# sair-lab/AirSLAM

Hardware: AMD Instinct MI355X
Metric: stereo detect+match pairs/sec (2x PLNet @512x512 internal: points + lines, junctions on the left + LightGlue match) (higher is better)
Workload: dtype fp16

## Files before the change

### airslam_amd/_lib.py

```python
from __future__ import annotations

import ctypes as C
import os

_HERE = os.path.dirname(os.path.abspath(__file__))
LIB_PATH = os.path.join(_HERE, "libairfe.so")


class Tuning(C.Structure):
    _fields_ = [(n, C.c_int) for n in (
        "fuse_lg_block", "gemm_small_max_m", "gemm8_min_m", "gemmr_min_m", "gemmr_wgs", "qkv_pair", "block_min_m", "lgb_tokens", "sg_kenc_gemm",
        "fold_qkv", "overlap_lines", "kf_graph", "kf_spec_rows", "fuse_dec", "assign_fused", "fold_out_proj", "desc_gather_stream", "copy_wgs")] + [("reserved", C.c_int * 5)]


class Cfg(C.Structure):
    _fields_ = [
        ("device", C.c_int), ("precision", C.c_int), ("max_batch", C.c_int), ("enc_chunk", C.c_int),
        ("max_keypoints", C.c_int), ("keypoint_threshold", C.c_float), ("remove_borders", C.c_int),
        ("nms_radius", C.c_int), ("line_threshold", C.c_float), ("line_length_threshold", C.c_float),
        ("matcher", C.c_int), ("image_width", C.c_int), ("image_height", C.c_int), ("sinkhorn_iters", C.c_int),
        ("superpoint_pack", C.c_char_p), ("plnet_s1_pack", C.c_char_p), ("lightglue_pack", C.c_char_p),
        ("superglue_pack", C.c_char_p), ("matcher_precision", C.c_int), ("line_precision", C.c_int), ("check_launches", C.c_int),
        ("tuning", C.POINTER(Tuning)),
    ]
# ... 262 lines not shown
    "airfe_debug_line_mid": (C.c_int, [C.c_void_p, C.POINTER(DebugLineMidArgs)]),
    "airfe_debug_s0_decode": (C.c_int, [C.c_void_p, C.POINTER(DebugS0DecodeArgs)]),
    "airfe_debug_lg_prepare": (C.c_int, [C.c_void_p, C.POINTER(DebugLgPrepareArgs)]),
    "airfe_debug_lg_assign": (C.c_int, [C.c_void_p, C.POINTER(DebugLgAssignArgs)]),
    "airfe_debug_plnet_stage0": (C.c_int, [C.c_void_p] + [C.c_void_p] * 10),
    "airfe_debug_plnet_s1": (C.c_int, [C.c_void_p, C.POINTER(Stage0), C.c_void_p, C.c_void_p, C.c_int, C.POINTER(C.c_int)]),
    "airfe_debug_plnet_s1_last": (C.c_int, [C.c_void_p, C.c_void_p, C.c_void_p, C.c_int, C.POINTER(C.c_int)]),
    "airfe_debug_preprocess": (C.c_int, [C.c_void_p, C.c_void_p, C.c_int, C.c_int, C.c_int, C.c_void_p]),
    "airfe_debug_conv3x3": (C.c_int, [C.c_void_p, C.c_void_p, C.c_int, C.c_int, C.c_int, C.c_int, C.c_void_p, C.c_void_p,
                                      C.c_int, C.c_int, C.c_void_p]),
    "airfe_debug_conv": (C.c_int, [C.c_void_p, C.POINTER(DebugConvArgs)]),
    "airfe_debug_trace": (C.c_int, [C.c_void_p, C.c_int]),
    "airfe_debug_trace_stop": (C.c_int, [C.c_void_p, C.c_int]),
    "airfe_debug_trace_buffer": (C.c_int, [C.c_void_p, C.c_int, C.c_void_p, C.c_size_t]),
    "airfe_debug_trace_slots": (C.c_int, [C.c_void_p]),
    "airfe_debug_trace_slot": (C.c_int, [C.c_void_p, C.c_int, C.c_char_p, C.c_int, C.POINTER(C.c_uint), C.POINTER(C.c_uint), C.POINTER(C.c_uint)]),
    "airfe_debug_trace_read": (C.c_int, [C.c_void_p, C.c_void_p, C.c_void_p, C.c_void_p]),
    "airfe_debug_gemm": (C.c_int, [C.c_void_p, C.c_void_p, C.c_int, C.c_int, C.c_void_p, C.c_void_p, C.c_int, C.c_int,
                                   C.c_void_p]),
    "airfe_debug_linear": (C.c_int, [C.c_void_p, C.POINTER(DebugLinearArgs)]),
    "airfe_debug_qkv": (C.c_int, [C.c_void_p] + [C.c_int] * 3 + [C.c_void_p] * 3 + [C.c_int] + [C.c_void_p] * 4 + [C.c_int] * 2 + [C.c_void_p] * 3),
    "airfe_debug_lg_block": (C.c_int, [C.c_void_p, C.POINTER(DebugLgBlockArgs)]),
    "airfe_debug_ln_gelu": (C.c_int, [C.c_void_p, C.c_int, C.c_void_p, C.c_void_p, C.c_void_p, C.c_int]),
    "airfe_debug_attention_args": (C.c_int, [C.c_void_p, C.POINTER(DebugAttentionArgs)]),
    "airfe_debug_attention": (C.c_int, [C.c_void_p, C.c_void_p, C.c_void_p, C.c_void_p, C.c_void_p, C.c_int, C.c_int, C.c_int, C.c_int, C.c_void_p]),
}

_lib = None


# ... 19 lines not shown
```

### airslam_amd/api.py

```python
from __future__ import annotations

import ctypes as C
import os
import tempfile
from typing import Dict, Optional

import numpy as np

from . import _lib, weights as W

FEAT = 259


def _pack_arg(x, tmpfiles) -> Optional[bytes]:
    if x is None:
        return None
    if isinstance(x, (str, bytes, os.PathLike)):
        return os.fsencode(x)
    f = tempfile.NamedTemporaryFile(suffix=".airfe", delete=False)
    f.close()
    W.save_pack(f.name, x)
    tmpfiles.append(f.name)
    return f.name.encode()


class AirfeError(RuntimeError):
    pass


class Context:

    def __init__(self, superpoint=None, lightglue=None, superglue=None, plnet_s1=None, tuning=None, **cfg):
        self._l = _lib.lib()
        c = _lib.Cfg()
        self._l.airfe_default_cfg(C.byref(c))
        t = None
        if tuning:
            t = _lib.Tuning()
            self._l.airfe_default_tuning(C.byref(t))
            for k, v in tuning.items():
                if k == "reserved" or not hasattr(t, k):
                    raise TypeError(f"unknown airfe_tuning field {k!r}")
                setattr(t, k, int(v))
            c.tuning = C.pointer(t)
        for k, v in cfg.items():
            if not hasattr(c, k):
                raise TypeError(f"unknown airfe_cfg field {k!r}")
            setattr(c, k, v)
        tmp = []
        try:
            c.superpoint_pack = _pack_arg(superpoint, tmp)
# ... 1296 lines not shown
```

### airslam_amd/csrc/airfe_debug.hip

```cpp
#include "airfe_host.h"

#include <memory>

struct HookStage {
  enum { OWN_TEXT = 1, SATURATION = 2, DEVICE_WIDE = 4 };
  HookStage(airfe_ctx* c_, const std::string& who_, int pack_prec = 0) : c(c_), who(who_), st(c_->stream) { mem.pack_prec = pack_prec; }
  HookStage(const HookStage&) = delete;
  ~HookStage() {
    if (queued) (void)hipStreamSynchronize(st);
    for (void* p : mem.allocs) (void)hipFree(p);
  }
  int status() const { return rc; }
  hipStream_t stream() { queued = true; return st; }
  int refuse(const std::string& m) { return rc ? rc : rc = fail(c, who + ": " + m); }
  void step(int r) { queued = true; if (r) rc = 1; }
  template <class T> T* fresh(size_t n, int byte) {
    T* p = raw<T>(n);
    fill(p, byte, std::max<size_t>(n, 1) * sizeof(T));
    return p;
  }
  template <class T> T* up(std::vector<T> v) { T* p = raw<T>(v.size()); put(p, std::move(v)); return p; }
  template <class T> T* up(const T* src, size_t n) { return up(std::vector<T>(src, src + n)); }
  bool linear(const float* W, const float* b, int K, int N, LinW& out) { if (!rc && !make_linear(&mem, W, b, K, N, out)) refuse("allocation failed"); return !rc; }
  void fill(void* p, int byte, size_t bytes) { if (!rc && bytes) hip(hipMemsetAsync(p, byte, bytes, stream()), "hipMemsetAsync"); }
// ... 174 lines not shown
  } else {
    g.X = s.up(dbg_conv_x(a->x, B, cin, H, W, prec));
  }
  g.Wp = s.up(dbg_conv_slabs(a->w, cin, cout, prec));
  g.bias = s.up(a->b, (size_t)cout);
  uint16_t* dy = s.fresh<uint16_t>(total, 0xFF);
  if (s.status()) return 1;
  g.Y = dy + guard;
  g.B = B; g.H = H; g.W = W; g.CIN = cin; g.COUT = cout; g.pool = pool; g.out_pad = opad; g.relu = a->relu; g.wgs = a->wgs;
  if (fused) launch_conv64r(prec, g, s.stream());
  else launch_conv3x3(prec, g, s.stream());
  s.wait(HookStage::OWN_TEXT);
  s.get(a->y_raw, dy, total * 2);
  return s.status();
} AIRFE_CATCH(c)

int airfe_debug_linear(airfe_ctx* c, const airfe_debug_linear_args* a) try {
  AIRFE_ENTER(c);
  if (!a || !a->x1 || !a->w || !a->b || !a->out) return fail(c, "debug_linear: null argument");
  const int prec = a->prec, M = a->M, K = a->K, N = a->N, epi = a->epi, kern = a->kernel, K1 = a->x2 ? a->K1 : K;
  if ((prec != 0 && prec != 1) || M < 1 || N < 1 || (K != 128 && K != 256 && K != 512) || K1 < 32 || K1 % 32 || K1 > K || (a->x2 && K1 == K) ||
      epi < EPI_STORE || epi > EPI_SOFTMAX_D2S || kern < AIRFE_DEBUG_KERNEL_DISPATCH || kern > AIRFE_DEBUG_KERNEL_GEMMR_GATHER128 || (a->act != ACT_NONE && a->act != ACT_RELU))
    return fail(c, "debug_linear: bad argument");
  const bool trans = epi == EPI_HEADS_T, heads = epi == EPI_HEADS || trans, d2s = epi == EPI_SOFTMAX_D2S;
  if (heads && ((a->H != 4 && a->H != 0) || a->Np < 16 || a->Np % 16 || M % a->Np || (epi == EPI_HEADS ? (N != 256 && N != 512) || (N == 512 && !a->out2) : N != 256)))
    return fail(c, "debug_linear: head layouts need H = 4, M = S * Np with Np a multiple of 16, N = 256 (or 512 with out2 for EPI_HEADS)");
  if ((a->rot_cos || a->rot_sin) && (epi != EPI_HEADS || !a->rot_cos || !a->rot_sin)) return fail(c, "debug_linear: rotary is an EPI_HEADS form");
  if (epi == EPI_RESID && (!a->x32 || N % 64)) return fail(c, "debug_linear: EPI_RESID needs x32 and N a multiple of 64");
  if (d2s && (K != 256 || N != 65 || a->x2 || a->rowidx || a->act || a->d2s_hc < 1 || a->d2s_wc < 1 || M % (a->d2s_hc * a->d2s_wc) || M % 16 ||
              (kern != AIRFE_DEBUG_KERNEL_DISPATCH && kern != AIRFE_DEBUG_KERNEL_GEMM8)))
// ... 890 lines not shown
```

### airslam_amd/csrc/common.h

```cpp
#pragma once
#include <hip/hip_runtime.h>
#include <stdint.h>
#include <atomic>
#include <mutex>

namespace airfe {

struct PerDeviceOnce {
  std::atomic<bool> done[64] = {};
  std::mutex mu;
  struct Token {
    PerDeviceOnce* owner = nullptr;
    int dev = 0;
    bool yes = false;
    std::unique_lock<std::mutex> lock;
    Token() = default;
    Token(Token&& o) noexcept : owner(o.owner), dev(o.dev), yes(o.yes), lock(std::move(o.lock)) { o.owner = nullptr; }
    Token(const Token&) = delete;
    Token& operator=(const Token&) = delete;
    explicit operator bool() const { return yes; }
    ~Token() { if (owner) owner->done[dev].store(true, std::memory_order_release); }
  };
  Token first() {
    Token t;
// ... 162 lines not shown
}

__device__ __forceinline__ void rotate_pairs(float* v, const f32x4& c, const f32x4& s) {
#pragma unroll
  for (int i = 0; i < 4; ++i) {
    float t0, t1, r0, r1;
    asm("v_mul_f32 %0, %1, %2" : "=v"(t0) : "v"(v[2 * i + 1]), "v"(s[i]));
    asm("v_fma_f32 %0, %1, %2, -%3" : "=v"(r0) : "v"(v[2 * i]), "v"(c[i]), "v"(t0));
    asm("v_mul_f32 %0, %1, %2" : "=v"(t1) : "v"(v[2 * i]), "v"(s[i]));
    asm("v_fma_f32 %0, %1, %2, %3" : "=v"(r1) : "v"(v[2 * i + 1]), "v"(c[i]), "v"(t1));
    v[2 * i] = r0;
    v[2 * i + 1] = r1;
  }
}

__device__ __forceinline__ void tile_decode(int tile, int per_img, int tiles_x, int sh_img, int sh_x, int& b, int& ty, int& tx) {
  if (sh_img >= 0) {
    b = tile >> sh_img;
    const int rem = tile & (per_img - 1);
    ty = rem >> sh_x;
    tx = rem & (tiles_x - 1);
  } else {
    b = tile / per_img;
    const int rem = tile - b * per_img;
    ty = rem / tiles_x;
    tx = rem - ty * tiles_x;
  }
}

__device__ __forceinline__ float wave_sum(float v) {
#pragma unroll
  for (int o = 32; o > 0; o >>= 1) v += __shfl_xor(v, o);
  return v;
}
__device__ __forceinline__ float wave_max(float v) {
#pragma unroll
  for (int o = 32; o > 0; o >>= 1) v = fmaxf(v, __shfl_xor(v, o));
  return v;
}

}
```

### airslam_amd/csrc/kernels.h

```cpp
#pragma once
#include <hip/hip_runtime.h>
#include <stdint.h>

namespace airfe {

enum Epi {
  EPI_STORE = 0,
  EPI_STORE_F32 = 1,
  EPI_RESID = 2,
  EPI_HEADS = 3,
  EPI_HEADS_T = 4,
  EPI_SOFTMAX_D2S = 5
};
enum Act { ACT_NONE = 0, ACT_RELU = 1 };

struct GemmArgs {
  const uint16_t* X1 = nullptr;
  const uint16_t* X2 = nullptr;
  int ld1 = 0, ld2 = 0, K1 = 0;
  const uint16_t* Wp = nullptr;
  const float* bias = nullptr;
  int M = 0;
  int N = 0;
  int cb_total = 0;
// ... 48 lines not shown
  const uint16_t* Wp = nullptr;
  const float* bias = nullptr;
  uint16_t* Y = nullptr;
  int B = 0, H = 0, W = 0, CIN = 0, COUT = 0;
  int pool = 0;
  int out_pad = 1;
  int relu = 1;
  int wgs = 256;
  const float* img = nullptr;
  const float* w1a = nullptr;
  const float* b1a = nullptr;
};
void launch_conv3x3(int prec, const ConvArgs& a, hipStream_t st);
void launch_conv64r(int prec, const ConvArgs& a, hipStream_t st);
void launch_conv128r(int prec, const ConvArgs& a, hipStream_t st);

void launch_preprocess(const uint8_t* src, int B, int h, int w, int stride, size_t img_stride,
                       const int* xtab , const int* ytab , const float* lut ,
                       float* out, int RH, int RW, hipStream_t st, const uint8_t* src1 = nullptr, int n0 = 0);

void launch_remap_linear(const uint8_t* src, int B, int h, int w, int stride, size_t img_stride, const float* mapx, const float* mapy,
                         uint8_t* dst, int dstride, size_t dimg_stride, hipStream_t st);

void launch_softmax_d2s(const float* logits, int ldl, float* heat, int B, int HC, int WC, hipStream_t st);
void launch_l2norm256(float* d, int rows, hipStream_t st);
void launch_simple_nms(const float* heat, float* out, float* tmp, int B, int H, int W, int radius, hipStream_t st);
void launch_nms512_candidates(const float* heat, float* out, void* planes, int B, float thr, int border, unsigned long long* cand,
                              int* cand_cnt, int cand_cap, hipStream_t st);
void launch_candidates(const float* heat, int B, int H, int W, float thr, int border, unsigned long long* cand,
                       int* cand_cnt, int cand_cap, hipStream_t st);
// ... 418 lines not shown
```

### airslam_amd/csrc/kernels_conv128r.hip

```cpp
#include "common.h"
#include "kernels.h"

namespace airfe {

typedef __attribute__((address_space(3))) void* las_ptr128r;

__device__ __forceinline__ void c128r_glds16(const void* gsrc, unsigned lds_off) {
  unsigned keep;
  asm volatile("s_mov_b32 %0, m0\n\ts_mov_b32 m0, %2\n\ts_nop 0\n\tglobal_load_lds_dwordx4 %1, off\n\ts_mov_b32 m0, %0"
               : "=&s"(keep)
               : "v"(gsrc), "s"(lds_off)
               : "memory");
}

constexpr int C128R_TILE_BYTES = 10 * 18 * 256;
constexpr int C128R_PIECES = 10 * 18 * 16;
constexpr int C128R_OUT_OFF = 2 * C128R_TILE_BYTES;
constexpr int C128R_LDS = C128R_OUT_OFF + 128 * 256;

template <class P, bool POOL>
__global__ __launch_bounds__(512, 1) void conv128r_kernel(ConvArgs a, int tiles_x, int tiles_y, int ntiles, int cb0) {
  extern __shared__ __attribute__((aligned(16))) char smem[];
  const int tid = threadIdx.x, lane = tid & 63, l15 = lane & 15, g = lane >> 4;
  const int wave = __builtin_amdgcn_readfirstlane(tid >> 6);
  const int cb = cb0 + (wave >> 2), t = wave & 3;
  const int H = a.H, W = a.W, COUT = a.COUT;
  const size_t in_row = (size_t)(W + 2) * 256;
  const size_t in_img = (size_t)(H + 2) * in_row;
  const int per_img = tiles_x * tiles_y;
  const unsigned lds_base = __builtin_amdgcn_readfirstlane((unsigned)(size_t)(las_ptr128r)smem);

  typename P::vec8 wreg[9][2][2];
  {
    const char* wp = reinterpret_cast<const char*>(a.Wp) + (size_t)cb * 18 * SLAB_BYTES;
    const int rr = t * 16 + l15;
#pragma unroll
    for (int tap = 0; tap < 9; ++tap)
#pragma unroll
      for (int cc = 0; cc < 2; ++cc)
#pragma unroll
        for (int ks = 0; ks < 2; ++ks) {
          const uint4 u = *reinterpret_cast<const uint4*>(wp + (tap * 2 + cc) * SLAB_BYTES + rr * 128 + (((ks * 4 + g) ^ swz128(rr)) << 4));
          wreg[tap][cc][ks] = __builtin_bit_cast(typename P::vec8, u);
        }
  }
  const int f0 = (t >> 1) * 32 + g * 8 + (t & 1) * 4;
  const f32x4 bias = *reinterpret_cast<const f32x4*>(a.bias + cb * 64 + f0);

  int goff[6];
#pragma unroll
  for (int j = 0; j < 6; ++j) {
    const int q = min(j * 512 + tid, C128R_PIECES - 1);
    const int p = q >> 4;
    const int pr = p / 18, pc = p - pr * 18;
    const int c = (q & 15) ^ (pc & 15);
    goff[j] = pr * (int)in_row + pc * 256 + c * 16;
  }
  const bool last_piece = 5 * 512 + tid < C128R_PIECES;
  auto stage_tile = [&](int tile, int buf) {
    const int b = tile / per_img, rem = tile - b * per_img;
    const int ty = rem / tiles_x, tx = rem - ty * tiles_x;
    const char* xin = reinterpret_cast<const char*>(a.X) + (size_t)b * in_img + (size_t)ty * 8 * in_row + (size_t)tx * 16 * 256;
    const unsigned dst = lds_base + buf * C128R_TILE_BYTES + wave * 1024;
#pragma unroll
    for (int j = 0; j < 5; ++j) c128r_glds16(xin + goff[j], dst + j * 8192);
    if (last_piece) c128r_glds16(xin + goff[5], dst + 5 * 8192);
  };
  int cbase[3];
#pragma unroll
  for (int dx = 0; dx < 3; ++dx) cbase[dx] = (l15 + dx) * 256 + ((g ^ ((l15 + dx) & 15)) << 4);

  const int Ho = POOL ? H / 2 : H, Wo = POOL ? W / 2 : W;
  const int opad = a.out_pad;
  const size_t orow = (size_t)(Wo + 2 * opad) * COUT;
  char* ost = smem + C128R_OUT_OFF;

  int tile = blockIdx.x;
  if (tile < ntiles) stage_tile(tile, 0);
  asm volatile("s_waitcnt vmcnt(0)" ::: "memory");
  __syncthreads();

  for (int i = 0; tile < ntiles; ++i, tile += gridDim.x) {
    const int next = tile + gridDim.x;
    if (next < ntiles) stage_tile(next, (i + 1) & 1);
    const int xoff = (i & 1) * C128R_TILE_BYTES;
    f32x4 acc[8];
#pragma unroll
    for (int m = 0; m < 8; ++m) acc[m] = bias;
#pragma unroll
    for (int c = 0; c < 12; ++c) {
      const int dx = c >> 2, cc = (c >> 1) & 1, ks = c & 1;
      typename P::vec8 bf[10];
      const char* fb = smem + ((cbase[dx] ^ (ks << 6) ^ (cc << 7)) + xoff);
#pragma unroll
      for (int r = 0; r < 10; ++r) bf[r] = lds_frag<P>(fb, r * (18 * 256));
#pragma unroll
      for (int dy = 0; dy < 3; ++dy)
#pragma unroll
        for (int m = 0; m < 8; ++m) acc[m] = P::mfma(wreg[dy * 3 + dx][cc][ks], bf[m + dy], acc[m]);
    }
    asm volatile("s_waitcnt vmcnt(0)" ::: "memory");
    __syncthreads();

    const int b = tile / per_img, rem = tile - b * per_img;
    const int ty = rem / tiles_x, tx = rem - ty * tiles_x;
    uint16_t* ybase = a.Y + (size_t)b * (Ho + 2 * opad) * orow + cb0 * 64;
    const int fch = (wave >> 2) * 8 + (f0 >> 3);
    uint2 pk[8];
#pragma unroll
    for (int m = 0; m < 8; ++m) pk[m] = uint2{P::pack2(acc[m][0], acc[m][1]), P::pack2(acc[m][2], acc[m][3])};
    if constexpr (!POOL) {
#pragma unroll
      for (int m = 0; m < 8; ++m) {
        const int px = m * 16 + l15;
        uint2 v = pk[m];
        if (a.relu) { v.x = relu_packed(v.x); v.y = relu_packed(v.y); }
        *reinterpret_cast<uint2*>(ost + px * 256 + ((fch ^ (px & 15)) << 4) + (t & 1) * 8) = v;
      }
      __syncthreads();
#pragma unroll
// ... 14 lines not shown
        if (a.relu) { v.x = relu_packed(v.x); v.y = relu_packed(v.y); }
        const int px = mp * 8 + (l15 >> 1);
        if (!(l15 & 1)) *reinterpret_cast<uint2*>(ost + px * 256 + ((fch ^ (px & 15)) << 4) + (t & 1) * 8) = v;
      }
      __syncthreads();
      {
        const int q = tid, px = q >> 4, c = q & 15;
        const uint4 v = *reinterpret_cast<const uint4*>(ost + px * 256 + ((c ^ (px & 15)) << 4));
        const int y = ty * 4 + (px >> 3), x = tx * 8 + (px & 7);
        *reinterpret_cast<uint4*>(ybase + (size_t)(y + opad) * orow + (size_t)(x + opad) * COUT + c * 8) = v;
      }
    }
  }
}

template <class P, bool POOL>
static void conv128r_launch_t(const ConvArgs& a, hipStream_t st) {
  static PerDeviceOnce attr_once;
  auto kfn = conv128r_kernel<P, POOL>;
  if (auto once_token = attr_once.first()) {
    (void)hipFuncSetAttribute(reinterpret_cast<const void*>(kfn), hipFuncAttributeMaxDynamicSharedMemorySize, C128R_LDS);
  }
  const int tiles_x = a.W / 16, tiles_y = a.H / 8;
  const int ntiles = tiles_x * tiles_y * a.B;
  const int grid = ntiles < a.wgs ? ntiles : a.wgs;
  for (int cb0 = 0; cb0 < a.COUT / 64; cb0 += 2)
    hipLaunchKernelGGL(kfn, dim3(grid), dim3(512), C128R_LDS, st, a, tiles_x, tiles_y, ntiles, cb0);
}

void launch_conv128r(int prec, const ConvArgs& a, hipStream_t st) {
  if (prec == 1) {
    if (a.pool) conv128r_launch_t<PF16, true>(a, st); else conv128r_launch_t<PF16, false>(a, st);
  } else {
    if (a.pool) conv128r_launch_t<PBF16, true>(a, st); else conv128r_launch_t<PBF16, false>(a, st);
  }
}

}
```

### airslam_amd/csrc/kernels_conv64r.hip

```cpp
#include "common.h"
#ifdef C64R_TIMING
__device__ long long c64_dbg[256 * 8 * 6];
#define C64R_T(x) { const long long now_ = wall_clock64(); x += now_ - tp_; tp_ = now_; }
#else
#define C64R_T(x)
#endif
#include "kernels.h"

namespace airfe {

typedef __attribute__((address_space(3))) void* las_ptr64r;

__device__ __forceinline__ void c64r_glds4(const void* gsrc, unsigned lds_off) {
  unsigned keep;
  asm volatile("s_mov_b32 %0, m0\n\ts_mov_b32 m0, %2\n\ts_nop 0\n\tglobal_load_lds_dword %1, off\n\ts_mov_b32 m0, %0"
               : "=&s"(keep)
               : "v"(gsrc), "s"(lds_off)
               : "memory");
}

__device__ __forceinline__ void c64r_glds16(const void* gsrc, unsigned lds_off) {
  unsigned keep;
  asm volatile("s_mov_b32 %0, m0\n\ts_mov_b32 m0, %2\n\ts_nop 0\n\tglobal_load_lds_dwordx4 %1, off\n\ts_mov_b32 m0, %0"
               : "=&s"(keep)
// ... 12 lines not shown
#endif
#ifndef C64R_RW
#define C64R_RW 4
#endif
#ifndef C64R_SPLIT_PROD
#define C64R_SPLIT_PROD 1
#endif
#ifndef C64R_EARLY_EPI
#define C64R_EARLY_EPI 1
#endif

constexpr int C64R_PATCH = 20 * 20;
constexpr int C64R_CONST_OFF = 2 * C64R_TILE_STRIDE + 3 * C64R_PATCH * 4;

template <class P, bool POOL, bool FUSE1A, int RW>
__global__ __launch_bounds__(2048 / RW, 1) void conv64r_kernel(ConvArgs a, int tiles_x, int tiles_y, int ntiles, int cb0) {
  extern __shared__ __attribute__((aligned(16))) char smem[];
  const int tid = threadIdx.x, lane = tid & 63, l15 = lane & 15, g = lane >> 4;
  const int wave = __builtin_amdgcn_readfirstlane(tid >> 6);
  constexpr bool CONST_IN_LDS = RW == 4;
  constexpr int NT = 2048 / RW;
  constexpr int NG = (21 * RW + 31) / 32;
  constexpr int NPC = (C64R_PIECES + NT - 1) / NT;
  const int ph = wave >> 1, ch = wave & 1;
  const int H = a.H, W = a.W, COUT = a.COUT;
  const size_t in_row = (size_t)(W + 2) * 128;
  const size_t in_img = (size_t)(H + 2) * in_row;
  const int per_img = tiles_x * tiles_y;
  const bool p2 = (tiles_x & (tiles_x - 1)) == 0 && (per_img & (per_img - 1)) == 0;
  const int sh_x = p2 ? __builtin_ctz(tiles_x) : -1, sh_img = p2 ? __builtin_ctz(per_img) : -1;

  typename P::vec8 wreg[9][2][2];
  {
    const char* wp = reinterpret_cast<const char*>(a.Wp) + (size_t)cb0 * 9 * SLAB_BYTES;
#pragma unroll
    for (int tap = 0; tap < 9; ++tap)
#pragma unroll
      for (int ks = 0; ks < 2; ++ks)
#pragma unroll
        for (int tt = 0; tt < 2; ++tt) {
          const int rr = (2 * ch + tt) * 16 + l15;
          const uint4 u = *reinterpret_cast<const uint4*>(wp + tap * SLAB_BYTES + rr * 128 + (((ks * 4 + g) ^ swz128(rr)) << 4));
          wreg[tap][ks][tt] = __builtin_bit_cast(typename P::vec8, u);
        }
  }
// ... 6 lines not shown
  const size_t orow = (size_t)(Wo + 2 * opad) * COUT;

  const unsigned lds_base = __builtin_amdgcn_readfirstlane((unsigned)(size_t)(las_ptr64r)smem);
  int goff[NPC];
#pragma unroll
  for (int j = 0; j < NPC; ++j) {
    const int q = min(j * NT + tid, C64R_PIECES - 1);
    const int p = q >> 3;
    const int pr = p / 18, pc = p - pr * 18;
    const int c = (q & 7) ^ ((pc >> 1) & 7);
    goff[j] = pr * (int)in_row + pc * 128 + c * 16;
  }
  const bool last_piece = (NPC - 1) * NT + tid < C64R_PIECES;
  auto stage = [&](int tile, int buf) {
    int b, ty, tx;
    tile_decode(tile, per_img, tiles_x, sh_img, sh_x, b, ty, tx);
    const char* xin = reinterpret_cast<const char*>(a.X) + (size_t)b * in_img + (size_t)ty * 16 * in_row + (size_t)tx * 16 * 128;
    const unsigned dst = lds_base + buf * C64R_TILE_STRIDE + wave * 1024;
#pragma unroll
    for (int j = 0; j < NPC - 1; ++j) c64r_glds16(xin + goff[j], dst + j * (NT * 16));
    if (last_piece) c64r_glds16(xin + goff[NPC - 1], dst + (NPC - 1) * (NT * 16));
  };
  int cbase[3];
#pragma unroll
  for (int dx = 0; dx < 3; ++dx) cbase[dx] = (ph * RW * 18 + l15 + dx) * 128 + ((g ^ (((l15 + dx) >> 1) & 7)) << 4);

  [[maybe_unused]] f16x8 w1[4];
  [[maybe_unused]] const unsigned pbase = lds_base + 2 * C64R_TILE_STRIDE;
  [[maybe_unused]] const float* pbuf = reinterpret_cast<const float*>(smem + 2 * C64R_TILE_STRIDE);
  if constexpr (FUSE1A) {
#pragma unroll
// ... 6 lines not shown
#pragma unroll
        for (int e = 0; e < 3; ++e) w[e] = (_Float16)a.w1a[co * 9 + g * 3 + e];
      } else {
        w[0] = (_Float16)a.b1a[co];
      }
      w1[t] = w;
      if constexpr (CONST_IN_LDS) { if (wave == 0) *reinterpret_cast<f16x8*>(smem + C64R_CONST_OFF + (t * 64 + lane) * 16) = w; }
    }
  }
  if constexpr (CONST_IN_LDS) {
#pragma unroll
    for (int e = 0; e < 8; ++e) reinterpret_cast<float*>(smem + C64R_CONST_OFF + 4096)[(ch * 4 + g) * 8 + e] = bias[e];
  }
  auto stage_patch = [&](int t, int buf) {
    int b, ty, tx;
    tile_decode(t, per_img, tiles_x, sh_img, sh_x, b, ty, tx);
    const float* img = a.img + (size_t)b * (H + 2) * (W + 2);
#pragma unroll
    for (int j = 0; j < (C64R_PATCH + NT - 1) / NT; ++j) {
      const int q = j * NT + tid;
      if (q < C64R_PATCH) {
        const int r = q / 20, cc = q - r * 20;
        const int gy = min(max(ty * 16 - 1 + r, 0), H + 1), gx = min(max(tx * 16 - 1 + cc, 0), W + 1);
        c64r_glds4(img + (size_t)gy * (W + 2) + gx, pbase + buf * (C64R_PATCH * 4) + (j * NT + wave * 64) * 4);
      }
    }
  };
  [[maybe_unused]] int prd[NG], pwr[NG], pyx[NG];
  if constexpr (FUSE1A) {
#pragma unroll
    for (int j = 0; j < NG; ++j) {
// ... 30 lines not shown
#pragma unroll
    for (int tp = 0; tp < 2; ++tp) {
      float v[8];
#pragma unroll
      for (int e = 0; e < 4; ++e) {
        v[e] = c1[2 * tp][e];
        v[4 + e] = c1[2 * tp + 1][e];
      }
      *reinterpret_cast<uint4*>(smem + xbuf * C64R_TILE_STRIDE + (pwr_j ^ (tp << 6))) = relu_packed(pack8<P>(v));
    }
  };
  auto prod_load = [&](int j, int buf) { return prod_load_at(prd[j], buf); };
  auto prod_finish = [&](int j, const Taps& tp3, int ty, int tx, int xbuf) { prod_finish_at(pwr[j], pyx[j], tp3, ty, tx, xbuf); };
  auto tile_xy = [&](int t, int& ty, int& tx) {
    int b_;
    tile_decode(t, per_img, tiles_x, sh_img, sh_x, b_, ty, tx);
  };

  int tile = blockIdx.x;
  if constexpr (FUSE1A) {
    if (tile < ntiles) stage_patch(tile, 0);
  } else {
    if (tile < ntiles) stage(tile, 0);
  }
  asm volatile("s_waitcnt vmcnt(0)" ::: "memory");
  __syncthreads();
  if constexpr (FUSE1A) {
    if (tile < ntiles) {
      if (tile + (int)gridDim.x < ntiles) stage_patch(tile + gridDim.x, 1);
      if (tile + 2 * (int)gridDim.x < ntiles) stage_patch(tile + 2 * gridDim.x, 2);
      int ty0, tx0;
      tile_xy(tile, ty0, tx0);
#pragma unroll
      for (int j = 0; j < NG; ++j) prod_finish(j, prod_load(j, 0), ty0, tx0, 0);
    }
    asm volatile("s_waitcnt vmcnt(0)" ::: "memory");
    __syncthreads();
  }

  int pb3 = 0, pb1 = 1;
#ifdef C64R_TIMING
  long long t_top = 0, t_mma = 0, t_wait = 0, t_bar = 0, t_epi = 0, tp_ = wall_clock64();
#endif
  for (int i = 0; tile < ntiles; ++i, tile += gridDim.x) {
    const int next = tile + gridDim.x;
    if constexpr (FUSE1A) {
      if (tile + 3 * (int)gridDim.x < ntiles) stage_patch(tile + 3 * gridDim.x, pb3);
    } else {
      if (next < ntiles) stage(next, (i + 1) & 1);
    }

    f32x4 acc[RW][2];
#pragma unroll
    for (int m = 0; m < RW; ++m)
#pragma unroll
      for (int t = 0; t < 2; ++t) {
        if constexpr (CONST_IN_LDS) acc[m][t] = *reinterpret_cast<const f32x4*>(smem + C64R_CONST_OFF + 4096 + (ch * 4 + g) * 32 + t * 16);
        else acc[m][t] = f32x4{bias[t * 4], bias[t * 4 + 1], bias[t * 4 + 2], bias[t * 4 + 3]};
      }
    constexpr bool PIN = RW == 4 && C64R_PIN;
    constexpr int NB = (RW == 8 || PIN) ? 2 : 1;
    typename P::vec8 bf[NB][RW + 2];
// ... 60 lines not shown
          if (prod_here) __builtin_amdgcn_sched_group_barrier(0x002, 5, 0);
        }
        if (prod_here) __builtin_amdgcn_sched_group_barrier(0x008, 6 * RW - 4 * (RW + 2) + 4, 0);
        else __builtin_amdgcn_sched_group_barrier(0x008, 6 * RW - 4 * (RW + 2), 0);
      }
    }
    if constexpr (SPLIT_PROD) {
      if (wave < 16 / RW) {
#pragma unroll
        for (int j = 0; j < NG; ++j) prod_finish(j, prod_load(j, pb1), nty, ntx, (i + 1) & 1);
      }
    }

    auto epilogue = [&]() {
    int b, ty, tx;
    tile_decode(tile, per_img, tiles_x, sh_img, sh_x, b, ty, tx);
    uint16_t* ybase = a.Y + (size_t)b * (Ho + 2 * opad) * orow + cb0 * 64 + ch * 32 + g * 8;
    uint4 pk[RW];
#pragma unroll
    for (int m = 0; m < RW; ++m) {
      pk[m].x = P::pack2(acc[m][0][0], acc[m][0][1]);
      pk[m].y = P::pack2(acc[m][0][2], acc[m][0][3]);
      pk[m].z = P::pack2(acc[m][1][0], acc[m][1][1]);
      pk[m].w = P::pack2(acc[m][1][2], acc[m][1][3]);
    }
    if constexpr (!POOL) {
#pragma unroll
      for (int m = 0; m < RW; ++m) {
        const int y = ty * 16 + ph * RW + m, x = tx * 16 + l15;
        *reinterpret_cast<uint4*>(ybase + (size_t)(y + opad) * orow + (size_t)(x + opad) * COUT) = relu_packed(pk[m]);
      }
// ... 6 lines not shown
          const uint4 vert = max_packed_pre_relu(pk[4 * q + 2 * h], pk[4 * q + 2 * h + 1]);
          v[h] = max_packed_pre_relu(vert, dpp_xor1(vert));
        }
        const uint4 r = relu_packed((l15 & 1) ? v[1] : v[0]);
        const int y = (ty * 16 + ph * RW) / 2 + 2 * q + (l15 & 1), x = tx * 8 + (l15 >> 1);
        *reinterpret_cast<uint4*>(ybase + (size_t)(y + opad) * orow + (size_t)(x + opad) * COUT) = r;
      }
    }
    };
    const bool early_epi = C64R_EARLY_EPI && wave < 16 / RW;
    if (early_epi) epilogue();
    C64R_T(t_mma)
    if constexpr (FUSE1A) {
      constexpr int NPP = (C64R_PATCH + NT - 1) / NT;
      constexpr int NST = POOL ? RW / 4 : RW;
      if (tile + 3 * (int)gridDim.x < ntiles) {
        if (early_epi) asm volatile("s_waitcnt vmcnt(%0) lgkmcnt(0)" ::"n"(NPP + NST) : "memory");
        else asm volatile("s_waitcnt vmcnt(%0) lgkmcnt(0)" ::"n"(NPP) : "memory");
      } else {
        if (early_epi) asm volatile("s_waitcnt vmcnt(%0) lgkmcnt(0)" ::"n"(NST) : "memory");
        else asm volatile("s_waitcnt vmcnt(0) lgkmcnt(0)" ::: "memory");
      }
      C64R_T(t_wait)
      __builtin_amdgcn_s_barrier();
      C64R_T(t_bar)
      pb3 = pb3 == 2 ? 0 : pb3 + 1;
      pb1 = pb1 == 2 ? 0 : pb1 + 1;
    } else {
      asm volatile("s_waitcnt vmcnt(0)" ::: "memory");
      __syncthreads();
    }
    if (!early_epi) epilogue();
    C64R_T(t_epi)
  }
#ifdef C64R_TIMING
  if (lane == 0 && FUSE1A) {
    long long* o = c64_dbg + (blockIdx.x * 8 + wave) * 6;
    o[0] = t_top; o[1] = t_mma; o[2] = t_wait; o[3] = t_bar; o[4] = t_epi;
  }
#endif
}

#ifdef C64R_TIMING
}
extern "C" int airfe_dbg_c64(long long* out) { return (int)hipMemcpyFromSymbol(out, HIP_SYMBOL(c64_dbg), sizeof(long long) * 256 * 8 * 6); }
namespace airfe {
#endif

template <class P, bool POOL, bool FUSE1A>
static void conv64r_launch_t(const ConvArgs& a, hipStream_t st) {
  constexpr int RW = C64R_RW;
  constexpr int LDS = C64R_CONST_OFF + 4096 + 256;
  static PerDeviceOnce attr_once;
  auto kfn = conv64r_kernel<P, POOL, FUSE1A, RW>;
  if (auto once_token = attr_once.first()) {
    (void)hipFuncSetAttribute(reinterpret_cast<const void*>(kfn), hipFuncAttributeMaxDynamicSharedMemorySize, LDS);
  }
  const int tiles_x = a.W / 16, tiles_y = a.H / 16;
  const int ntiles = tiles_x * tiles_y * a.B;
  const int grid = ntiles < a.wgs ? ntiles : a.wgs;
  for (int cb0 = 0; cb0 < a.COUT / 64; ++cb0)
    hipLaunchKernelGGL(kfn, dim3(grid), dim3(2048 / RW), LDS, st, a, tiles_x, tiles_y, ntiles, cb0);
}

void launch_conv64r(int prec, const ConvArgs& a, hipStream_t st) {
  if (a.img) {
    if (prec == 1) conv64r_launch_t<PF16, true, true>(a, st); else conv64r_launch_t<PBF16, true, true>(a, st);
    return;
  }
  if (prec == 1) {
    if (a.pool) conv64r_launch_t<PF16, true, false>(a, st); else conv64r_launch_t<PF16, false, false>(a, st);
  } else {
    if (a.pool) conv64r_launch_t<PBF16, true, false>(a, st); else conv64r_launch_t<PBF16, false, false>(a, st);
  }
}

}
// ... 1 lines not shown
```

### airslam_amd/csrc/kernels_mm.hip

```cpp
#include <cstdlib>

#include "common.h"
#include "kernels.h"

namespace airfe {

template <int CIN>
__device__ __forceinline__ int swz_pix(int p) {
  if constexpr (CIN == 64) return swz128(p);
  else return swz256(p);
}

template <class P, int CIN, int MR, bool POOL>
__global__ __launch_bounds__(256) void conv3x3_kernel(ConvArgs a, int tiles_x, int tiles_y, int cb_per_block) {
  constexpr int TH = 4 * MR, TW = 16, PH = TH + 2, PW = TW + 2;
  constexpr int PIXB = CIN * 2, CPP = CIN / 8, NS = 9 * (CIN / 64);
  constexpr int TILE_BYTES = PH * PW * PIXB;
  extern __shared__ __attribute__((aligned(16))) char smem[];
  char* xs = smem;
  char* ws = smem + TILE_BYTES;

  const int tid = threadIdx.x, lane = tid & 63, wave = tid >> 6, l15 = lane & 15, g = lane >> 4;
  const int bid = blockIdx.x;
  const int tx = bid % tiles_x, ty = (bid / tiles_x) % tiles_y, b = bid / (tiles_x * tiles_y);
// ... 125 lines not shown
  const int cbt = a.COUT / 64;
  const long blocks = (long)tiles_x * tiles_y * a.B;
  const int gy = (blocks >= 2048) ? 1 : cbt;
  dim3 grid((unsigned)blocks, (unsigned)gy);
  hipLaunchKernelGGL(kfn, grid, dim3(256), LDS, st, a, tiles_x, tiles_y, cbt / gy);
}

template <class P>
static void conv_launch_p(const ConvArgs& a, hipStream_t st) {
  if (a.CIN == 64) {
    if (a.pool) conv_launch_t<P, 64, 4, true>(a, st); else conv_launch_t<P, 64, 4, false>(a, st);
  } else {
    if (a.pool) conv_launch_t<P, 128, 2, true>(a, st); else conv_launch_t<P, 128, 2, false>(a, st);
  }
}

void launch_conv3x3(int prec, const ConvArgs& a, hipStream_t st) {
  if (a.CIN == 64 && (a.COUT % 64) == 0 && a.relu && (a.H % 16) == 0 && (a.W % 16) == 0) {
    launch_conv64r(prec, a, st);
    return;
  }
  if (a.CIN == 128 && (a.COUT % 128) == 0 && a.relu && (a.H % 8) == 0 && (a.W % 16) == 0) {
    launch_conv128r(prec, a, st);
    return;
  }
  if (prec == 1) conv_launch_p<PF16>(a, st); else conv_launch_p<PBF16>(a, st);
}

template <class P>
__device__ __forceinline__ void gemm_store_run(const GemmArgs& a, int row, int co0, float* v) {
// ... 268 lines not shown
```

### include/airfe_debug.h

```cpp
#ifndef AIRFE_DEBUG_H_
#define AIRFE_DEBUG_H_
#include "airfe.h"
#ifdef __cplusplus
extern "C" {
#endif

int airfe_debug_detector_maps(airfe_ctx* ctx, int B, float* heat_raw, float* heat_nms, float* desc);
int airfe_debug_lightglue_scores(airfe_ctx* ctx, const float* f0, int n0, const float* f1, int n1, float* scores);
int airfe_debug_lg_filter(airfe_ctx* ctx, const float* scores, int n0, int n1, int32_t* idx, float* score, int cap, int* nmatch);
int airfe_debug_sg_decode(airfe_ctx* ctx, const float* Z, int n0, int n1, int32_t* idx0, int32_t* idx1, double* ms0, double* ms1);
int airfe_debug_sg_sinkhorn(airfe_ctx* ctx, const float* sim, const int* lens , int B, int ld ,
                            float alpha, int iters, int form , float* Z , int* form_ran);
int airfe_debug_superglue_scores(airfe_ctx* ctx, const float* f0, int n0, const float* f1, int n1, float* scores);
int airfe_debug_plnet_stage0(airfe_ctx* ctx, float* juncs_pred, float* lines_pred, float* iskeep, float* idx_min, float* idx_max,
                             float* loi, float* thin, float* aux, float* jloc, float* joff);
int airfe_debug_plnet_j2l(airfe_ctx* ctx, int fast, float* iskeep, float* idx_min, float* idx_max);
int airfe_debug_plnet_s1(airfe_ctx* ctx, const airfe_plnet_stage0* stage0, float* lines_adjusted, float* scores_line,
                         int cap, int* m2);
int airfe_debug_plnet_s1_last(airfe_ctx* ctx, float* lines_adjusted, float* scores_line, int cap, int* m2);
int airfe_debug_preprocess(airfe_ctx* ctx, const uint8_t* gray, int h, int w, int stride, float* out);
int airfe_debug_conv3x3(airfe_ctx* ctx, const float* x, int B, int cin, int H, int W, const float* w, const float* b,
                        int cout, int pool, float* y);
int airfe_debug_gemm(airfe_ctx* ctx, const float* x, int M, int K, const float* w, const float* b, int N, int relu, float* y);
typedef struct airfe_debug_conv_args {
  const float* x;
  const float* img;
  const float *w1a, *b1a;
  const float *w, *b;
  int cin, cout, B, H, W;
  int pool, out_pad, relu, wgs;
  size_t y_words;
  uint16_t* y_raw;
} airfe_debug_conv_args;
int airfe_debug_conv(airfe_ctx* ctx, airfe_debug_conv_args* a);
enum {
  AIRFE_DEBUG_KERNEL_DISPATCH = 0,
  AIRFE_DEBUG_KERNEL_SMALL = 1,
  AIRFE_DEBUG_KERNEL_TILED = 2,
  AIRFE_DEBUG_KERNEL_GEMM8 = 3,
  AIRFE_DEBUG_KERNEL_GEMMR = 4,
  AIRFE_DEBUG_KERNEL_GEMMR_GATHER = 5,
  AIRFE_DEBUG_KERNEL_GEMMR_GATHER128 = 6
};
typedef struct airfe_debug_linear_args {
  int prec, M, K, K1, N;
  const float* x1;
  const float* x2;
  const float* w;
  const float* b;
// ... 172 lines not shown
```

Before: 8062.

## Merge conv output-channel passes into one launch with XCD-aware blocked tile order

The 64r and 128r conv kernels used to be launched once per output-channel block, walking tiles in raster order. They now launch once, and each workgroup picks its channel pass and tile from its index. Workgroups on the same XCD (8 assumed) get spatially contiguous 2D tile blocks, so neighbouring tiles and halos share that XCD's L2. This removes extra launches and aims to improve cache locality. It adds index arithmetic and a global runtime switch (default on) to choose the ordering.

```diff
diff --git a/airslam_amd/_lib.py b/airslam_amd/_lib.py
--- a/airslam_amd/_lib.py
+++ b/airslam_amd/_lib.py
@@ -300,6 +300,7 @@
     "airfe_debug_trace_stop": (C.c_int, [C.c_void_p, C.c_int]),
     "airfe_debug_trace_buffer": (C.c_int, [C.c_void_p, C.c_int, C.c_void_p, C.c_size_t]),
     "airfe_debug_trace_slots": (C.c_int, [C.c_void_p]),
+    "airfe_debug_conv_order": (C.c_int, [C.c_int, C.POINTER(C.c_int)]),
     "airfe_debug_trace_slot": (C.c_int, [C.c_void_p, C.c_int, C.c_char_p, C.c_int, C.POINTER(C.c_uint), C.POINTER(C.c_uint), C.POINTER(C.c_uint)]),
     "airfe_debug_trace_read": (C.c_int, [C.c_void_p, C.c_void_p, C.c_void_p, C.c_void_p]),
     "airfe_debug_gemm": (C.c_int, [C.c_void_p, C.c_void_p, C.c_int, C.c_int, C.c_void_p, C.c_void_p, C.c_int, C.c_int,
diff --git a/airslam_amd/api.py b/airslam_amd/api.py
--- a/airslam_amd/api.py
+++ b/airslam_amd/api.py
@@ -28,6 +28,13 @@
     pass
 
 
+def conv_tile_order(order: int) -> int:
+    prev = C.c_int()
+    if _lib.lib().airfe_debug_conv_order(int(order), C.byref(prev)) != 0:
+        raise AirfeError((_lib.lib().airfe_last_error(None) or b"airfe_debug_conv_order failed").decode())
+    return prev.value
+
+
 class Context:
 
     def __init__(self, superpoint=None, lightglue=None, superglue=None, plnet_s1=None, tuning=None, **cfg):
@@ -35,6 +42,9 @@
         c = _lib.Cfg()
         self._l.airfe_default_cfg(C.byref(c))
         t = None
+        if tuning and "conv_order" in tuning:
+            tuning = dict(tuning)
+            conv_tile_order(int(tuning.pop("conv_order")))
         if tuning:
             t = _lib.Tuning()
             self._l.airfe_default_tuning(C.byref(t))
diff --git a/airslam_amd/csrc/airfe_debug.hip b/airslam_amd/csrc/airfe_debug.hip
--- a/airslam_amd/csrc/airfe_debug.hip
+++ b/airslam_amd/csrc/airfe_debug.hip
@@ -212,6 +212,13 @@
   s.get(a->y_raw, dy, total * 2);
   return s.status();
 } AIRFE_CATCH(c)
+
+int airfe_debug_conv_order(int order, int* previous) try {
+  if (order < -1 || order > CONV_ORDER_DEFAULT) return fail(nullptr, "debug_conv_order: order must lie in -1 .. 3");
+  const int before = conv_tile_order_switch(order);
+  if (previous) *previous = before;
+  return 0;
+} AIRFE_CATCH(nullptr)
 
 int airfe_debug_linear(airfe_ctx* c, const airfe_debug_linear_args* a) try {
   AIRFE_ENTER(c);
diff --git a/airslam_amd/csrc/common.h b/airslam_amd/csrc/common.h
--- a/airslam_amd/csrc/common.h
+++ b/airslam_amd/csrc/common.h
@@ -200,20 +200,6 @@
   }
 }
 
-__device__ __forceinline__ void tile_decode(int tile, int per_img, int tiles_x, int sh_img, int sh_x, int& b, int& ty, int& tx) {
-  if (sh_img >= 0) {
-    b = tile >> sh_img;
-    const int rem = tile & (per_img - 1);
-    ty = rem >> sh_x;
-    tx = rem & (tiles_x - 1);
-  } else {
-    b = tile / per_img;
-    const int rem = tile - b * per_img;
-    ty = rem / tiles_x;
-    tx = rem - ty * tiles_x;
-  }
-}
-
 __device__ __forceinline__ float wave_sum(float v) {
 #pragma unroll
   for (int o = 32; o > 0; o >>= 1) v += __shfl_xor(v, o);
diff --git a/airslam_amd/csrc/conv_tile_order.h b/airslam_amd/csrc/conv_tile_order.h
--- /dev/null
+++ b/airslam_amd/csrc/conv_tile_order.h
@@ -0,0 +1,102 @@
+#pragma once
+
+#if defined(__HIPCC__)
+#define AIRFE_CTO_HD __host__ __device__ __forceinline__
+#else
+#define AIRFE_CTO_HD inline
+#endif
+
+namespace airfe {
+
+constexpr int CONV_XCDS = 8;
+
+struct ConvTileOrder {
+  int tiles_x = 0, per_img = 0, ntiles = 0;
+  int passes = 1, sh_pass = 0;
+  int pass0 = 0;
+  int chunk = 0;
+  int sh_img = -1, sh_x = -1;
+  int sh_bw = 0, sh_blk = 0;
+};
+
+AIRFE_CTO_HD bool conv_pow2(int v) { return v > 0 && (v & (v - 1)) == 0; }
+AIRFE_CTO_HD int conv_log2(int v) {
+  int s = 0;
+  while ((1 << (s + 1)) <= v) ++s;
+  return s;
+}
+
+AIRFE_CTO_HD ConvTileOrder conv_tile_order(int order, int grid, int tiles_x, int tiles_y, int images, int passes, int tile_w, int tile_h) {
+  ConvTileOrder o;
+  o.tiles_x = tiles_x;
+  o.per_img = tiles_x * tiles_y;
+  o.ntiles = o.per_img * images;
+  const bool p2 = conv_pow2(tiles_x) && conv_pow2(tiles_y);
+  if (p2) {
+    o.sh_x = conv_log2(tiles_x);
+    o.sh_img = conv_log2(o.per_img);
+    o.sh_bw = o.sh_x;
+    o.sh_blk = o.sh_x;
+  }
+  const int per_xcd = grid / CONV_XCDS;
+  if (!order || grid < CONV_XCDS || grid % CONV_XCDS || !conv_pow2(passes) || per_xcd % passes) return o;
+  o.passes = passes;
+  o.sh_pass = conv_log2(passes);
+  o.chunk = per_xcd / passes;
+  if (p2) {
+    int bw = 1, bh = 1;
+    while (bw * bh * 2 <= o.chunk) {
+      const bool gx = bw * 2 <= tiles_x, gy = bh * 2 <= tiles_y;
+      if (gx && (bw * tile_w <= bh * tile_h || !gy)) bw *= 2;
+      else if (gy) bh *= 2;
+      else break;
+    }
+    o.sh_bw = conv_log2(bw);
+    o.sh_blk = conv_log2(bw * bh);
+  }
+  return o;
+}
+AIRFE_CTO_HD int conv_tile_launches(const ConvTileOrder& o, int passes) { return o.chunk ? 1 : passes; }
+
+AIRFE_CTO_HD void conv_tile_first(const ConvTileOrder& o, int wg, int grid, int& first, int& step, int& pass) {
+  if (o.chunk) {
+    const int x = wg & (CONV_XCDS - 1), s = wg >> 3;
+    first = x * o.chunk + (s >> o.sh_pass);
+    step = CONV_XCDS * o.chunk;
+    pass = o.pass0 + (s & (o.passes - 1));
+  } else {
+    first = wg;
+    step = grid;
+    pass = o.pass0;
+  }
+}
+
+AIRFE_CTO_HD void conv_tile_decode_shift(const ConvTileOrder& o, int tile, int& b, int& ty, int& tx) {
+  b = tile >> o.sh_img;
+  const int rem = tile & (o.per_img - 1);
+  const int blk = rem >> o.sh_blk, w = rem & ((1 << o.sh_blk) - 1);
+  const int sh_bx = o.sh_x - o.sh_bw, sh_bh = o.sh_blk - o.sh_bw;
+  ty = ((blk >> sh_bx) << sh_bh) + (w >> o.sh_bw);
+  tx = ((blk & ((1 << sh_bx) - 1)) << o.sh_bw) + (w & ((1 << o.sh_bw) - 1));
+}
+AIRFE_CTO_HD void conv_tile_decode_div(const ConvTileOrder& o, int tile, int& b, int& ty, int& tx) {
+  b = tile / o.per_img;
+  const int rem = tile - b * o.per_img;
+  ty = rem / o.tiles_x;
+  tx = rem - ty * o.tiles_x;
+}
+AIRFE_CTO_HD void conv_tile_decode(const ConvTileOrder& o, int tile, int& b, int& ty, int& tx) {
+  if (o.sh_img >= 0) conv_tile_decode_shift(o, tile, b, ty, tx);
+  else conv_tile_decode_div(o, tile, b, ty, tx);
+}
+
+AIRFE_CTO_HD bool conv_tile_map(const ConvTileOrder& o, int wg, int i, int grid, int& pass, int& b, int& ty, int& tx) {
+  int first, step;
+  conv_tile_first(o, wg, grid, first, step, pass);
+  const long long tile = (long long)first + (long long)i * step;
+  if (tile >= o.ntiles) return false;
+  conv_tile_decode(o, (int)tile, b, ty, tx);
+  return true;
+}
+
+}
diff --git a/airslam_amd/csrc/kernels.h b/airslam_amd/csrc/kernels.h
--- a/airslam_amd/csrc/kernels.h
+++ b/airslam_amd/csrc/kernels.h
@@ -86,6 +86,9 @@
 void launch_conv3x3(int prec, const ConvArgs& a, hipStream_t st);
 void launch_conv64r(int prec, const ConvArgs& a, hipStream_t st);
 void launch_conv128r(int prec, const ConvArgs& a, hipStream_t st);
+constexpr int CONV_ORDER_64R = 1, CONV_ORDER_128R = 2, CONV_ORDER_DEFAULT = CONV_ORDER_64R | CONV_ORDER_128R;
+int conv_tile_order_switch();
+int conv_tile_order_switch(int v);
 
 void launch_preprocess(const uint8_t* src, int B, int h, int w, int stride, size_t img_stride,
                        const int* xtab , const int* ytab , const float* lut ,
diff --git a/airslam_amd/csrc/kernels_conv128r.hip b/airslam_amd/csrc/kernels_conv128r.hip
--- a/airslam_amd/csrc/kernels_conv128r.hip
+++ b/airslam_amd/csrc/kernels_conv128r.hip
@@ -1,4 +1,5 @@
 #include "common.h"
+#include "conv_tile_order.h"
 #include "kernels.h"
 
 namespace airfe {
@@ -18,16 +19,18 @@
 constexpr int C128R_OUT_OFF = 2 * C128R_TILE_BYTES;
 constexpr int C128R_LDS = C128R_OUT_OFF + 128 * 256;
 
-template <class P, bool POOL>
-__global__ __launch_bounds__(512, 1) void conv128r_kernel(ConvArgs a, int tiles_x, int tiles_y, int ntiles, int cb0) {
+template <class P, bool POOL, bool SHIFT>
+__global__ __launch_bounds__(512, 1) void conv128r_kernel(ConvArgs a, ConvTileOrder o) {
   extern __shared__ __attribute__((aligned(16))) char smem[];
   const int tid = threadIdx.x, lane = tid & 63, l15 = lane & 15, g = lane >> 4;
   const int wave = __builtin_amdgcn_readfirstlane(tid >> 6);
+  int tile, tstep, pass;
+  conv_tile_first(o, blockIdx.x, gridDim.x, tile, tstep, pass);
+  const int ntiles = o.ntiles, cb0 = 2 * pass;
   const int cb = cb0 + (wave >> 2), t = wave & 3;
   const int H = a.H, W = a.W, COUT = a.COUT;
   const size_t in_row = (size_t)(W + 2) * 256;
   const size_t in_img = (size_t)(H + 2) * in_row;
-  const int per_img = tiles_x * tiles_y;
   const unsigned lds_base = __builtin_amdgcn_readfirstlane((unsigned)(size_t)(las_ptr128r)smem);
 
   typename P::vec8 wreg[9][2][2];
@@ -58,8 +61,8 @@
   }
   const bool last_piece = 5 * 512 + tid < C128R_PIECES;
   auto stage_tile = [&](int tile, int buf) {
-    const int b = tile / per_img, rem = tile - b * per_img;
-    const int ty = rem / tiles_x, tx = rem - ty * tiles_x;
+    int b, ty, tx;
+    if constexpr (SHIFT) conv_tile_decode_shift(o, tile, b, ty, tx); else conv_tile_decode_div(o, tile, b, ty, tx);
     const char* xin = reinterpret_cast<const char*>(a.X) + (size_t)b * in_img + (size_t)ty * 8 * in_row + (size_t)tx * 16 * 256;
     const unsigned dst = lds_base + buf * C128R_TILE_BYTES + wave * 1024;
 #pragma unroll
@@ -75,13 +78,12 @@
   const size_t orow = (size_t)(Wo + 2 * opad) * COUT;
   char* ost = smem + C128R_OUT_OFF;
 
-  int tile = blockIdx.x;
   if (tile < ntiles) stage_tile(tile, 0);
   asm volatile("s_waitcnt vmcnt(0)" ::: "memory");
   __syncthreads();
 
-  for (int i = 0; tile < ntiles; ++i, tile += gridDim.x) {
-    const int next = tile + gridDim.x;
+  for (int i = 0; tile < ntiles; ++i, tile += tstep) {
+    const int next = tile + tstep;
     if (next < ntiles) stage_tile(next, (i + 1) & 1);
     const int xoff = (i & 1) * C128R_TILE_BYTES;
     f32x4 acc[8];
@@ -102,8 +104,8 @@
     asm volatile("s_waitcnt vmcnt(0)" ::: "memory");
     __syncthreads();
 
-    const int b = tile / per_img, rem = tile - b * per_img;
-    const int ty = rem / tiles_x, tx = rem - ty * tiles_x;
+    int b, ty, tx;
+    if constexpr (SHIFT) conv_tile_decode_shift(o, tile, b, ty, tx); else conv_tile_decode_div(o, tile, b, ty, tx);
     uint16_t* ybase = a.Y + (size_t)b * (Ho + 2 * opad) * orow + cb0 * 64;
     const int fch = (wave >> 2) * 8 + (f0 >> 3);
     uint2 pk[8];
@@ -148,18 +150,26 @@
   }
 }
 
-template <class P, bool POOL>
-static void conv128r_launch_t(const ConvArgs& a, hipStream_t st) {
+template <class P, bool POOL, bool SHIFT>
+static void conv128r_launch_k(const ConvArgs& a, ConvTileOrder o, int grid, int launches, hipStream_t st) {
   static PerDeviceOnce attr_once;
-  auto kfn = conv128r_kernel<P, POOL>;
+  auto kfn = conv128r_kernel<P, POOL, SHIFT>;
   if (auto once_token = attr_once.first()) {
     (void)hipFuncSetAttribute(reinterpret_cast<const void*>(kfn), hipFuncAttributeMaxDynamicSharedMemorySize, C128R_LDS);
   }
+  for (; o.pass0 < launches; ++o.pass0) hipLaunchKernelGGL(kfn, dim3(grid), dim3(512), C128R_LDS, st, a, o);
+}
+
+template <class P, bool POOL>
+static void conv128r_launch_t(const ConvArgs& a, hipStream_t st) {
   const int tiles_x = a.W / 16, tiles_y = a.H / 8;
   const int ntiles = tiles_x * tiles_y * a.B;
   const int grid = ntiles < a.wgs ? ntiles : a.wgs;
-  for (int cb0 = 0; cb0 < a.COUT / 64; cb0 += 2)
-    hipLaunchKernelGGL(kfn, dim3(grid), dim3(512), C128R_LDS, st, a, tiles_x, tiles_y, ntiles, cb0);
+  const int passes = a.COUT / 128;
+  const ConvTileOrder o = conv_tile_order(conv_tile_order_switch() & CONV_ORDER_128R, grid, tiles_x, tiles_y, a.B, passes, 16, 8);
+  const int launches = conv_tile_launches(o, passes);
+  if (o.sh_img >= 0) conv128r_launch_k<P, POOL, true>(a, o, grid, launches, st);
+  else conv128r_launch_k<P, POOL, false>(a, o, grid, launches, st);
 }
 
 void launch_conv128r(int prec, const ConvArgs& a, hipStream_t st) {
diff --git a/airslam_amd/csrc/kernels_conv64r.hip b/airslam_amd/csrc/kernels_conv64r.hip
--- a/airslam_amd/csrc/kernels_conv64r.hip
+++ b/airslam_amd/csrc/kernels_conv64r.hip
@@ -5,6 +5,7 @@
 #else
 #define C64R_T(x)
 #endif
+#include "conv_tile_order.h"
 #include "kernels.h"
 
 namespace airfe {
@@ -50,7 +51,7 @@
 constexpr int C64R_CONST_OFF = 2 * C64R_TILE_STRIDE + 3 * C64R_PATCH * 4;
 
 template <class P, bool POOL, bool FUSE1A, int RW>
-__global__ __launch_bounds__(2048 / RW, 1) void conv64r_kernel(ConvArgs a, int tiles_x, int tiles_y, int ntiles, int cb0) {
+__global__ __launch_bounds__(2048 / RW, 1) void conv64r_kernel(ConvArgs a, ConvTileOrder o) {
   extern __shared__ __attribute__((aligned(16))) char smem[];
   const int tid = threadIdx.x, lane = tid & 63, l15 = lane & 15, g = lane >> 4;
   const int wave = __builtin_amdgcn_readfirstlane(tid >> 6);
@@ -62,9 +63,9 @@
   const int H = a.H, W = a.W, COUT = a.COUT;
   const size_t in_row = (size_t)(W + 2) * 128;
   const size_t in_img = (size_t)(H + 2) * in_row;
-  const int per_img = tiles_x * tiles_y;
-  const bool p2 = (tiles_x & (tiles_x - 1)) == 0 && (per_img & (per_img - 1)) == 0;
-  const int sh_x = p2 ? __builtin_ctz(tiles_x) : -1, sh_img = p2 ? __builtin_ctz(per_img) : -1;
+  int tile, tstep, cb0;
+  conv_tile_first(o, blockIdx.x, gridDim.x, tile, tstep, cb0);
+  const int ntiles = o.ntiles;
 
   typename P::vec8 wreg[9][2][2];
   {
@@ -101,7 +102,7 @@
   const bool last_piece = (NPC - 1) * NT + tid < C64R_PIECES;
   auto stage = [&](int tile, int buf) {
     int b, ty, tx;
-    tile_decode(tile, per_img, tiles_x, sh_img, sh_x, b, ty, tx);
+    conv_tile_decode(o, tile, b, ty, tx);
     const char* xin = reinterpret_cast<const char*>(a.X) + (size_t)b * in_img + (size_t)ty * 16 * in_row + (size_t)tx * 16 * 128;
     const unsigned dst = lds_base + buf * C64R_TILE_STRIDE + wave * 1024;
 #pragma unroll
@@ -138,7 +139,7 @@
   }
   auto stage_patch = [&](int t, int buf) {
     int b, ty, tx;
-    tile_decode(t, per_img, tiles_x, sh_img, sh_x, b, ty, tx);
+    conv_tile_decode(o, t, b, ty, tx);
     const float* img = a.img + (size_t)b * (H + 2) * (W + 2);
 #pragma unroll
     for (int j = 0; j < (C64R_PATCH + NT - 1) / NT; ++j) {
@@ -199,10 +200,9 @@
   auto prod_finish = [&](int j, const Taps& tp3, int ty, int tx, int xbuf) { prod_finish_at(pwr[j], pyx[j], tp3, ty, tx, xbuf); };
   auto tile_xy = [&](int t, int& ty, int& tx) {
     int b_;
-    tile_decode(t, per_img, tiles_x, sh_img, sh_x, b_, ty, tx);
+    conv_tile_decode(o, t, b_, ty, tx);
   };
 
-  int tile = blockIdx.x;
   if constexpr (FUSE1A) {
     if (tile < ntiles) stage_patch(tile, 0);
   } else {
@@ -212,8 +212,8 @@
   __syncthreads();
   if constexpr (FUSE1A) {
     if (tile < ntiles) {
-      if (tile + (int)gridDim.x < ntiles) stage_patch(tile + gridDim.x, 1);
-      if (tile + 2 * (int)gridDim.x < ntiles) stage_patch(tile + 2 * gridDim.x, 2);
+      if (tile + tstep < ntiles) stage_patch(tile + tstep, 1);
+      if (tile + 2 * tstep < ntiles) stage_patch(tile + 2 * tstep, 2);
       int ty0, tx0;
       tile_xy(tile, ty0, tx0);
 #pragma unroll
@@ -227,10 +227,10 @@
 #ifdef C64R_TIMING
   long long t_top = 0, t_mma = 0, t_wait = 0, t_bar = 0, t_epi = 0, tp_ = wall_clock64();
 #endif
-  for (int i = 0; tile < ntiles; ++i, tile += gridDim.x) {
-    const int next = tile + gridDim.x;
+  for (int i = 0; tile < ntiles; ++i, tile += tstep) {
+    const int next = tile + tstep;
     if constexpr (FUSE1A) {
-      if (tile + 3 * (int)gridDim.x < ntiles) stage_patch(tile + 3 * gridDim.x, pb3);
+      if (tile + 3 * tstep < ntiles) stage_patch(tile + 3 * tstep, pb3);
     } else {
       if (next < ntiles) stage(next, (i + 1) & 1);
     }
@@ -321,7 +321,7 @@
 
     auto epilogue = [&]() {
     int b, ty, tx;
-    tile_decode(tile, per_img, tiles_x, sh_img, sh_x, b, ty, tx);
+    conv_tile_decode(o, tile, b, ty, tx);
     uint16_t* ybase = a.Y + (size_t)b * (Ho + 2 * opad) * orow + cb0 * 64 + ch * 32 + g * 8;
     uint4 pk[RW];
 #pragma unroll
@@ -358,7 +358,7 @@
     if constexpr (FUSE1A) {
       constexpr int NPP = (C64R_PATCH + NT - 1) / NT;
       constexpr int NST = POOL ? RW / 4 : RW;
-      if (tile + 3 * (int)gridDim.x < ntiles) {
+      if (tile + 3 * tstep < ntiles) {
         if (early_epi) asm volatile("s_waitcnt vmcnt(%0) lgkmcnt(0)" ::"n"(NPP + NST) : "memory");
         else asm volatile("s_waitcnt vmcnt(%0) lgkmcnt(0)" ::"n"(NPP) : "memory");
       } else {
@@ -379,8 +379,8 @@
   }
 #ifdef C64R_TIMING
   if (lane == 0 && FUSE1A) {
-    long long* o = c64_dbg + (blockIdx.x * 8 + wave) * 6;
-    o[0] = t_top; o[1] = t_mma; o[2] = t_wait; o[3] = t_bar; o[4] = t_epi;
+    long long* dbg = c64_dbg + (blockIdx.x * 8 + wave) * 6;
+    dbg[0] = t_top; dbg[1] = t_mma; dbg[2] = t_wait; dbg[3] = t_bar; dbg[4] = t_epi;
   }
 #endif
 }
@@ -403,8 +403,10 @@
   const int tiles_x = a.W / 16, tiles_y = a.H / 16;
   const int ntiles = tiles_x * tiles_y * a.B;
   const int grid = ntiles < a.wgs ? ntiles : a.wgs;
-  for (int cb0 = 0; cb0 < a.COUT / 64; ++cb0)
-    hipLaunchKernelGGL(kfn, dim3(grid), dim3(2048 / RW), LDS, st, a, tiles_x, tiles_y, ntiles, cb0);
+  const int passes = a.COUT / 64;
+  ConvTileOrder o = conv_tile_order(conv_tile_order_switch() & CONV_ORDER_64R, grid, tiles_x, tiles_y, a.B, passes, 16, 16);
+  for (const int n = conv_tile_launches(o, passes); o.pass0 < n; ++o.pass0)
+    hipLaunchKernelGGL(kfn, dim3(grid), dim3(2048 / RW), LDS, st, a, o);
 }
 
 void launch_conv64r(int prec, const ConvArgs& a, hipStream_t st) {
diff --git a/airslam_amd/csrc/kernels_mm.hip b/airslam_amd/csrc/kernels_mm.hip
--- a/airslam_amd/csrc/kernels_mm.hip
+++ b/airslam_amd/csrc/kernels_mm.hip
@@ -163,6 +163,10 @@
     if (a.pool) conv_launch_t<P, 128, 2, true>(a, st); else conv_launch_t<P, 128, 2, false>(a, st);
   }
 }
+
+static std::atomic<int> g_conv_order{CONV_ORDER_DEFAULT};
+int conv_tile_order_switch() { return g_conv_order.load(std::memory_order_relaxed); }
+int conv_tile_order_switch(int v) { return g_conv_order.exchange(v < 0 ? CONV_ORDER_DEFAULT : (v & CONV_ORDER_DEFAULT), std::memory_order_relaxed); }
 
 void launch_conv3x3(int prec, const ConvArgs& a, hipStream_t st) {
   if (a.CIN == 64 && (a.COUT % 64) == 0 && a.relu && (a.H % 16) == 0 && (a.W % 16) == 0) {
diff --git a/include/airfe_debug.h b/include/airfe_debug.h
--- a/include/airfe_debug.h
+++ b/include/airfe_debug.h
@@ -33,6 +33,7 @@
   uint16_t* y_raw;
 } airfe_debug_conv_args;
 int airfe_debug_conv(airfe_ctx* ctx, airfe_debug_conv_args* a);
+int airfe_debug_conv_order(int order, int* previous);
 enum {
   AIRFE_DEBUG_KERNEL_DISPATCH = 0,
   AIRFE_DEBUG_KERNEL_SMALL = 1,
```

After: 8177 (median of 6 runs). 1.01x the previous value.
